# tsbertalan/openmg

Hardware: AMD Instinct MI355X
Metric: V-cycles/sec, 3-D 7-point Poisson 256^3 (higher is better)
Workload: dtype f64

## Files before the change

### include/openmg_hip.h

```cpp
#ifndef OPENMG_HIP_H
#define OPENMG_HIP_H

#include <stdint.h>

#ifdef __cplusplus
extern "C" {
#endif

#define OMG_OK                0
#define OMG_ERR_INVALID       1
#define OMG_ERR_NO_DEVICE     2
#define OMG_ERR_HIP           3
#define OMG_ERR_SINGULAR      4
#define OMG_ERR_NO_DIAGONAL   5
#define OMG_ERR_ALLOC         6
#define OMG_ERR_UNSUPPORTED   7

#define OMG_SMOOTH_GS_LEX     0
#define OMG_SMOOTH_GS_COLOUR  1
#define OMG_SMOOTH_JACOBI     2

typedef struct {
    int64_t n_rows, n_cols, nnz;
    const int32_t *indptr;
// ... 6 lines not shown

const char *omg_last_error(void);
int omg_device_count(int *count);
int omg_set_device(int device);
int omg_device_mem_info(int64_t *free_bytes, int64_t *total_bytes);
int omg_device_synchronize(void);
const char *omg_version(void);

int omg_hierarchy_create(int n_levels, const omg_csr *A, const omg_csr *R,
                         int smoother, double omega, omg_hierarchy **out);
#define OMG_DTYPE_F64 0
#define OMG_DTYPE_F32 1
int omg_hierarchy_create_ex(int n_levels, const omg_csr *A, const omg_csr *R, int smoother,
                            double omega, int dtype, omg_hierarchy **out);
int omg_hierarchy_create_from_fine(const omg_csr *A_in, int dim, const int64_t *shape, int n_restrictions, int smoother, double omega,
                                   int dtype, omg_hierarchy **out);

int omg_hierarchy_update_fine(omg_hierarchy *h, const double *data, int64_t nnz, int on_device);
int omg_hierarchy_dtype(const omg_hierarchy *h, int *dtype);
int omg_hierarchy_destroy(omg_hierarchy *h);
int omg_hierarchy_set_stream(omg_hierarchy *h, void *hip_stream);
int omg_hierarchy_sync(omg_hierarchy *h);
int omg_hierarchy_level_rows(const omg_hierarchy *h, int level, int64_t *n_rows);
int omg_hierarchy_level_sets(const omg_hierarchy *h, int level, int64_t *n_sets);
int omg_hierarchy_level_fused(const omg_hierarchy *h, int level, int *fused);
#define OMG_LEVEL_FUSED_LAST_SET   1
#define OMG_LEVEL_SCATTER_PROLONG  2
#define OMG_LEVEL_UNION_WALK       16
#define OMG_LEVEL_MARCH            32
#define OMG_LEVEL_MARCH_SCAN       512
#define OMG_LEVEL_PLANE            64
#define OMG_LEVEL_VAR7             256
#define OMG_LEVEL_STENCIL27        128
int omg_hierarchy_level_flags(const omg_hierarchy *h, int level, int *flags);
int omg_hierarchy_use_plane(omg_hierarchy *h, int enable);
int omg_hierarchy_plane_info(const omg_hierarchy *h, int level, int64_t *out8);
int omg_hierarchy_set_info(const omg_hierarchy *h, int level, int set, int64_t *rows, int64_t *nnz);
#define OMG_FORMAT_FIELDS 12
int omg_hierarchy_format_info(const omg_hierarchy *h, int level, int op, int set, int64_t *out);
int omg_format_selftest(const omg_csr *A, int dtype, int64_t *out);

int omg_vcycle(omg_hierarchy *h, int level, const double *b, double *x,
               int pre, int post, double *norm);
int omg_vcycle_ex(omg_hierarchy *h, int level, const double *b, const double *x_in, double *x_out, double *x_pre,
                  int pre, int post, double *norm);

int omg_solve(omg_hierarchy *h, const double *b, double *x, int pre, int post,
              int max_cycles, double threshold, int *cycles_done, double *norm);

int omg_vcycle_dev(omg_hierarchy *h, int level, const double *b_dev, const double *x_in_dev, double *x_out_dev,
                   double *x_pre_dev, int pre, int post, double *norm);
int omg_resident_load_dev(omg_hierarchy *h, const double *b_dev, const double *x0_dev );
int omg_resident_fetch_dev(omg_hierarchy *h, double *x_dev);

int omg_hierarchy_cycle_dev(omg_hierarchy *h, const double *b_dev, double *x_dev, int pre, int post,
                            void *hip_stream);

int omg_resident_load(omg_hierarchy *h, const double *b, const double *x0 );
int omg_resident_cycle(omg_hierarchy *h, int pre, int post, double *norm );
int omg_resident_cycles(omg_hierarchy *h, int pre, int post, int n_cycles, double *norms );
int omg_resident_fetch(omg_hierarchy *h, double *x);
int omg_resident_spmv_time(omg_hierarchy *h, int reps, double *avg_ms);
int omg_resident_use_graph(omg_hierarchy *h, int enable);

#define OMG_PROFILE_CLASSES 7
int omg_profile_enable(omg_hierarchy *h, int mask);
// ... 135 lines not shown
```

### openmg_amd/_hip.py

```python
import ctypes
import os

import numpy as np
import scipy.sparse as sp

_HERE = os.path.dirname(os.path.abspath(__file__))
LIB_PATH = os.environ.get("OMG_LIB_PATH") or os.path.join(_HERE, "lib", "libopenmg_hip.so")

OMG_OK = 0
ERR_INVALID, ERR_NO_DEVICE, ERR_HIP, ERR_SINGULAR, ERR_NO_DIAGONAL, ERR_ALLOC, ERR_UNSUPPORTED = range(1, 8)
SMOOTH_GS_LEX, SMOOTH_GS_COLOUR, SMOOTH_JACOBI = 0, 1, 2
PROFILE_CLASSES = 7
PROFILE_NAMES = ("smoother_set_sweep", "residual", "restrict", "prolong_add", "residual_norm", "plane_down", "plane_up")

SMOOTHERS = {
    "gs": SMOOTH_GS_LEX, "lex": SMOOTH_GS_LEX, "gauss-seidel": SMOOTH_GS_LEX, "gaussSeidel": SMOOTH_GS_LEX,
    "colour": SMOOTH_GS_COLOUR, "color": SMOOTH_GS_COLOUR, "rbgs": SMOOTH_GS_COLOUR,
    "red-black": SMOOTH_GS_COLOUR, "multicolour": SMOOTH_GS_COLOUR,
    "jacobi": SMOOTH_JACOBI, "weighted-jacobi": SMOOTH_JACOBI,
}


class HipError(RuntimeError):

# ... 385 lines not shown
        ms = ctypes.c_double(0.0)
        check(lib().omg_resident_spmv_time(self._h, int(reps), ctypes.byref(ms)))
        return ms.value

    def use_graph(self, enable=True):
        check(lib().omg_resident_use_graph(self._h, 1 if enable else 0))

    def set_stream(self, hip_stream):
        check(lib().omg_hierarchy_set_stream(self._h, ctypes.c_void_p(hip_stream or 0)))

    def sync(self):
        check(lib().omg_hierarchy_sync(self._h))

    def device_dtype(self):
        code = ctypes.c_int(-1)
        check(lib().omg_hierarchy_dtype(self._h, ctypes.byref(code)))
        return np.dtype(np.float32 if code.value == DTYPE_F32 else np.float64)

    def level_sets(self, level):
        v = ctypes.c_int64(0)
        check(lib().omg_hierarchy_level_sets(self._h, level, ctypes.byref(v)))
        return v.value

    def level_fused(self, level):
        v = ctypes.c_int(0)
        check(lib().omg_hierarchy_level_fused(self._h, level, ctypes.byref(v)))
        return bool(v.value)

    def level_flags(self, level):
        f = ctypes.c_int(0)
        check(lib().omg_hierarchy_level_flags(self._h, int(level), ctypes.byref(f)))
        return {"fused_last_set": bool(f.value & 1), "scatter_prolong": bool(f.value & 2), "union_walk": bool(f.value & 16),
                "march": bool(f.value & 32), "plane": bool(f.value & 64), "stencil27": bool(f.value & 128), "var7": bool(f.value & 256),
                "march_scan": bool(f.value & 512)}

    def use_plane(self, enable=True):
        check(lib().omg_hierarchy_use_plane(self._h, 1 if enable else 0))

    PLANE_FIELDS = ("nx", "ny", "nz", "tile_x", "tile_y", "tile_z", "workgroups", "threads")

    def plane_info(self, level):
        out = (ctypes.c_int64 * len(self.PLANE_FIELDS))()
        check(lib().omg_hierarchy_plane_info(self._h, int(level), out))
        return dict(zip(self.PLANE_FIELDS, [int(v) for v in out]))

    def set_info(self, level, s):
        rows, nnz = ctypes.c_int64(0), ctypes.c_int64(0)
        check(lib().omg_hierarchy_set_info(self._h, level, s, ctypes.byref(rows), ctypes.byref(nnz)))
        return rows.value, nnz.value

    FORMAT_FIELDS = ("rows", "nnz", "blocks", "pattern_blocks", "pattern_rows", "pattern_nnz",
                     "coldict_nnz", "valdict_nnz", "format_bytes", "csr_bytes", "ell_blocks", "ell_nnz")

    def format_info(self, level, op="A", set=-1):
        out = (ctypes.c_int64 * len(self.FORMAT_FIELDS))()
        check(lib().omg_hierarchy_format_info(self._h, int(level), {"A": 0, "R": 1, "P": 2}[op], int(set), out))
        return dict(zip(self.FORMAT_FIELDS, [int(v) for v in out]))

    def profile_enable(self, classes=True):
        if classes is True:
            mask = -1
        elif not classes:
            mask = 0
        else:
            mask = 0
            for name in classes:
                mask |= 1 << PROFILE_NAMES.index(name)
# ... 147 lines not shown
```

### openmg_amd/csrc/common.h

```cpp
#pragma once
#include <hip/hip_runtime.h>

#include <cstdint>
#include <cstdio>
#include <cstdlib>
#include <stdexcept>
#include <memory>
#include <string>
#include <utility>
#include <vector>

#include "../../include/openmg_hip.h"

#if !defined(OMG_EXPERIMENTS) && (defined(PLANE_STORE_AUX) || defined(PLANE_LA_BIG) || defined(PLANE_LA) || defined(PLANE_WAVE_SYNC) || \
                                  defined(PLANE_WSYNC_F32) || defined(S27_COEF_AUX) || defined(S27_SG) || defined(S27_WAVES) ||        \
                                  defined(MARCH_NAP_MAX) || defined(OMG_ROWBLK_NNZ) || defined(PLANE_SETPRIO))
#error "tuning switches are experiments: add -DOMG_EXPERIMENTS"
#endif

namespace omg {

inline const char *experiment_env(const char *name) {
#ifdef OMG_EXPERIMENTS
    return getenv(name);
// ... 373 lines not shown
    bool build(const omg_csr &A, hipStream_t s);
    void sweep(V *x, const V *b, hipStream_t s) const;
    bool timed_out(hipStream_t s) const;
};

struct DevCsrPlain {
    int64_t n_rows = 0, n_cols = 0, nnz = 0;
    DevBuf<int32_t> indptr, indices;
    DevBuf<double> data;
};
void galerkin_chain_device(const omg_csr &A0, int dim, const int64_t *shape, int n_restrictions, std::vector<DevCsrPlain> &A,
                           std::vector<DevCsrPlain> &R, hipStream_t s);
HostCsr download_csr(const DevCsrPlain &M, hipStream_t s);
bool rap_aggregation_device(const DevCsrPlain &R, const DevCsrPlain &A, DevCsrPlain &C, hipStream_t s);

bool is_plain_aggregation(const omg_csr &R, int64_t nx, int64_t ny, int64_t nz, double &w);

constexpr int PLANE_EDGE = 4;
struct PlaneGeom {
    int nx = 0, ny = 0, nz = 0;
    int hx = 0;
    int z_base = 0, z_end = 0, kv0 = 0, kv1 = 0, kc_off = 0, nzc = 0;
    int TX = 0, TY = 0, LZ = 0;
    int PX = 0, PY = 0;
    int ntx = 0, nty = 0, ntz = 0, n_wg = 0;
    int threads = 0;
    size_t lds_bytes = 0;
    double c[7] = {0, 0, 0, 0, 0, 0, 0};
    double w = 0.0;
    bool dim2 = false;
    bool jacobi = false;
    double omega = 1.0;
    bool block = false;
    bool la2 = true;
};
template <typename V>
struct PlanePlan {
    PlaneGeom g;
    DevBuf<double> partials;
    uint32_t *status = nullptr;
    bool build(const omg_csr &A, const omg_csr &R, Ordering &ord, bool jacobi = false, double omega = 1.0);
    bool build_device(const DevCsrPlain &A, int nx, int ny, int nz, double w, Ordering &ord, bool jacobi, double omega, hipStream_t s);
    bool finish_geometry(int64_t nx, int64_t ny, int64_t nz, const double (&c)[7], double w, bool jacobi, double omega);
    void spmv(const V *x, V *y, hipStream_t s) const;
    HostCsr operator_csr() const;
    HostCsr restriction_csr() const;
    void build_slab(int nx, int ny, int nz_own, int ghost, int ghost_c, bool first, bool last, const double (&c)[7], double w);
    struct Peer {
        V *x[2] = {nullptr, nullptr};
        V *bc[2] = {nullptr, nullptr};
        int64_t shift = 0, cshift = 0;
        int planes = 0, cplanes = 0;
        int zc_lo = 0, zc_hi = 0;
        const uint32_t *wait_flag[4] = {nullptr, nullptr, nullptr, nullptr};
        uint32_t wait_seq[4] = {0, 0, 0, 0};
        bool fused_wait = true;
        uint32_t *done = nullptr;
        uint32_t *flag[2] = {nullptr, nullptr};
        uint32_t seq = 0;
        uint32_t *status = nullptr;
        uint32_t spin = 1u << 21;
    };
    struct Coarse {
        const int32_t *map = nullptr;
        V *b = nullptr;
        V *x = nullptr;
        const V *diag = nullptr;
        int first_end = 0;
        const V *e = nullptr;
    };
    void tune(V *x, V *tmp, const V *b, const Coarse &c, hipStream_t s, bool finest = true);
    float time_pair(V *x, V *tmp, const V *b, const Coarse &c, hipStream_t s, bool finest, int pairs);
    enum { PART_ALL = 0, PART_EDGE = 1, PART_INNER = 2 };
    bool can_split() const {
        return !g.dim2 && !g.block && !(g.la2 && g.threads <= 128) && (g.z_end - g.z_base) >= 3 * PLANE_EDGE;
    }
    int split_partials() const {
        const int nzo = g.z_end - g.z_base;
        return nzo >= 3 * PLANE_EDGE ? g.ntx * g.nty * (2 + (nzo - 2 * PLANE_EDGE + g.LZ - 1) / g.LZ) : g.n_wg;
    }
    struct Gate {
        const uint32_t *flag[4] = {nullptr, nullptr, nullptr, nullptr};
        uint32_t seq[4] = {0, 0, 0, 0};
        uint32_t *status = nullptr;
        uint32_t spin = 1u << 21;
    };
    bool can_gate() const { return can_split() && 2 * g.ntx * g.nty <= 192 && (g.z_end - g.z_base) >= 96; }
    int gate_lz() const;
    int gate_partials() const;
    void down(const V *x_old, V *x_new, const V *b, bool x_zero, const Coarse &c, hipStream_t s, const Peer *peer = nullptr,
              bool sweep = true, int part = PART_ALL, const Gate *gate = nullptr) const;
    void up(const V *x_old, V *x_new, const V *b, const Coarse &c, double *out, hipStream_t s, const Peer *peer = nullptr,
            bool sweep = true, int part = PART_ALL, const Gate *gate = nullptr) const;
};

template <typename V>
struct Var7Plan {
    int nx = 0, ny = 0, nz = 0;
    double w = 0.0;
    bool sym = false;
    int tx = 0, ty = 0, lz = 0, ntx = 0, nty = 0, ntz = 0, threads = 0;
    int64_t n_wg = 0;
    DevBuf<V> cD, cM[3], cP[3];
    DevBuf<double> partials;
// ... 51 lines not shown
```

### openmg_amd/csrc/hierarchy.hip

```cpp
#include <algorithm>
#include <chrono>
#include <cmath>
#include <cstring>
#include <memory>
#include <array>
#include <map>
#include <mutex>
#include <thread>
#include <type_traits>

#include "common.h"

namespace omg {

std::vector<ScatteredBlock> &scattered_registry() {
    static std::vector<ScatteredBlock> r;
    return r;
}
static std::mutex &scattered_mutex() {
    static std::mutex m;
    return m;
}
static void scattered_release(ScatteredBlock &blk, size_t mapped) {
    auto report = [](const char *what, hipError_t e) {
// ... 1544 lines not shown
        with(h, [&](auto *hh) {
            check_level(hh, level);
            OMG_REQUIRE(n_sets, "null");
            *n_sets = (int64_t)hh->lv[level].ord.sets.size() - 1;
        });
    });
}

int omg_hierarchy_level_fused(const omg_hierarchy *h, int level, int *fused) {
    return guarded([&] {
        with(h, [&](auto *hh) {
            check_level(hh, level);
            OMG_REQUIRE(fused, "null");
            ensure_format(hh, level);
            *fused = (level + 1 < (int)hh->lv.size() && can_fuse(hh, hh->lv[level])) ? 1 : 0;
        });
    });
}

int omg_hierarchy_level_flags(const omg_hierarchy *h, int level, int *flags) {
    return guarded([&] {
        with(h, [&](auto *hh) {
            check_level(hh, level);
            OMG_REQUIRE(flags, "null");
            ensure_format(hh, level);
            const bool smoothed = level + 1 < (int)hh->lv.size();
            *flags = ((smoothed && can_fuse(hh, hh->lv[level])) ? OMG_LEVEL_FUSED_LAST_SET : 0) |
                     ((smoothed && hh->lv[level].scatter_prolong) ? OMG_LEVEL_SCATTER_PROLONG : 0) |
                     ((smoothed && hh->lv[level].A.all_union()) ? OMG_LEVEL_UNION_WALK : 0) |
                     ((smoothed && hh->lv[level].march) ? OMG_LEVEL_MARCH : 0) |
                     ((smoothed && hh->lv[level].march && hh->lv[level].march->line_scan) ? OMG_LEVEL_MARCH_SCAN : 0) |
                     ((smoothed && hh->lv[level].plane && !hh->no_plane) ? OMG_LEVEL_PLANE : 0) |
                     ((smoothed && hh->lv[level].s27 && !hh->no_plane) ? OMG_LEVEL_STENCIL27 : 0) |
                     ((smoothed && hh->lv[level].var7 && !hh->no_plane) ? OMG_LEVEL_VAR7 : 0);
        });
    });
}

int omg_hierarchy_use_plane(omg_hierarchy *h, int enable) {
    return guarded([&] {
        with(h, [&](auto *hh) {
            OMG_HIP(hipStreamSynchronize(hh->stream));
            drop_graph(hh);
            hh->no_plane = enable == 0;
        });
    });
}

int omg_hierarchy_plane_info(const omg_hierarchy *h, int level, int64_t *out8) {
    return guarded([&] {
        with(h, [&](auto *hh) {
            check_level(hh, level);
            OMG_REQUIRE(out8, "null");
            for (int i = 0; i < 8; ++i) out8[i] = 0;
            const auto &L = hh->lv[level];
            if (!L.plane) return;
            const PlaneGeom &g = L.plane->g;
            const int64_t v[8] = {g.nx, g.ny, g.nz, g.TX, g.TY, g.LZ, g.n_wg, g.threads};
            for (int i = 0; i < 8; ++i) out8[i] = v[i];
        });
    });
}

int omg_hierarchy_set_info(const omg_hierarchy *h, int level, int set, int64_t *rows, int64_t *nnz) {
    return guarded([&] {
        with(h, [&](auto *hh) {
            check_level(hh, level);
// ... 690 lines not shown
```

### openmg_amd/csrc/plane.hip

```cpp
#include <algorithm>
#include <array>
#include <atomic>
#include <cmath>
#include <cstring>
#include <map>
#include <mutex>
#include <thread>
#include <type_traits>

#include "common.h"

#if defined(OMG_PLANE_STAMPS) || defined(OMG_PLANE_DBGARGS)
#define OMG_PLANE_DBG_ON 1
#endif

namespace omg {
namespace {

#ifndef PLANE_STORE_AUX
#define PLANE_STORE_AUX 2
#endif
typedef unsigned v2u __attribute__((ext_vector_type(2)));
typedef unsigned v4u __attribute__((ext_vector_type(4)));
typedef int v2i __attribute__((ext_vector_type(2)));
// ... 1029 lines not shown
            E[c] = B[l] - row(l);
            if (SWEEP) a.x_new[slot_of(gi, gj, gk)] = X[l];
        }
        __syncthreads();
#pragma unroll
        for (int n = 0; n < NC; ++n) {
            const int c = t + n * NT;
            if (cs[n] < 0) continue;
            const int I = c % hx, J = (c / hx) % hy, K = c / (hx * hy);
            V acc = V(0);
#pragma unroll
            for (int d = 0; d < 8; ++d)
                acc = madd(a.w, E[((2 * K + (d >> 2)) * BY + 2 * J + ((d >> 1) & 1)) * BX + 2 * I + (d & 1)], acc);
            a.bc[cs[n]] = acc;
        }
    } else {
        if (SWEEP) {
            sweep(0, R1(), std::false_type());
            __syncthreads();
            sweep(1, R0(), std::false_type());
            __syncthreads();
        }
#pragma unroll
        for (int n = 0; n < NB; ++n) {
            const int c = t + n * NT;
            const int li = 2 + c % BX, lj = 2 + (c / BX) % BY, lk = 2 + c / (BX * BY);
            const int gi = i0 + li, gj = j0 + lj, gk = k0 + lk;
            if (c >= BX * BY * BZ || gi >= a.nx || gj >= a.ny || gk >= a.nz) continue;
            a.x_new[slot_of(gi, gj, gk)] = X[(lk * EY + lj) * EX + li];
        }
    }
}

template <typename V>
struct Tile2KArgs {
    const V *x_old;
    V *x_new;
    const V *b;
    int nx, ny, nr;
    int nbx;
    V c1, c2, c3, c4, c5, w, omega;
    int fast_div;
    int nxc, nyc;
    const int32_t *cmap;
    V *bc;
    const V *ec;
    double *partials;
};

template <typename V, int MODE, bool XZ, bool NORM, bool SWEEP, int BX, int BY, bool JAC = false>
__global__ __launch_bounds__(256) void tile2d_kernel(const Tile2KArgs<V> a) {
    extern __shared__ __attribute__((aligned(16))) unsigned char plane_smem[];
    constexpr int EX = BX + 6, EY = BY + 6, vol = EX * EY, NT = 256;
    V *const X = reinterpret_cast<V *>(plane_smem);
    V *const B = X + vol;
    V *const XN = B + vol;
    V *const E = JAC ? XN + vol : XN;
    __shared__ double s_red[NT / 64];
    const int t = int(threadIdx.x);
    const int bi = int(blockIdx.x) % a.nbx, bj = int(blockIdx.x) / a.nbx;
    const int i0 = bi * BX - 3, j0 = bj * BY - 3;
    const V rc3 = refined_rcp(a.c3);
    const bool fast = a.fast_div != 0;
    auto slot_of = [&](int gi, int gj) { return JAC ? gj * a.nx + gi : (((gi + gj) & 1) ? a.nr : 0) + ((gj * a.nx + gi) >> 1); };
    auto in_grid = [&](int gi, int gj) { return gi >= 0 && gi < a.nx && gj >= 0 && gj < a.ny; };
    constexpr int NL = (vol + NT - 1) / NT;
// ... 102 lines not shown
        for (int n = 0; n < NCC; ++n) {
            const int c = t + n * NT;
            const int I = c % hx, J = c / hx;
            const int GI = (bi * BX >> 1) + I, GJ = (bj * BY >> 1) + J;
            if (c >= hx * hy || GI >= a.nxc || GJ >= a.nyc) continue;
            V acc = V(0);
#pragma unroll
            for (int d = 0; d < 4; ++d) acc = madd(a.w, E[(2 * J + (d >> 1)) * BX + 2 * I + (d & 1)], acc);
            const int ce = GJ * a.nxc + GI;
            a.bc[a.cmap ? a.cmap[ce] : ce] = acc;
        }
    }
    if (NORM) {
#pragma unroll
        for (int off = 32; off > 0; off >>= 1) sq += __shfl_down(sq, off, 64);
        if ((t & 63) == 0) s_red[t >> 6] = sq;
        __syncthreads();
        if (t == 0) {
            double tot = 0.0;
            for (int wv = 0; wv < NT / 64; ++wv) tot += s_red[wv];
            a.partials[blockIdx.x] = tot;
        }
    }
}

int env_int3(const char *name, int out[3]) {
    const char *e = getenv(name);
    if (!e || !e[0]) return 0;
    return sscanf(e, "%d,%d,%d", &out[0], &out[1], &out[2]) == 3 ? 1 : 0;
}

inline int round_up(int v, int m) { return (v + m - 1) / m * m; }

inline void small_level_switches(PlaneGeom &g) {
    auto env = [](const char *name, long long dflt) { const char *e = getenv(name); return e && e[0] ? atoll(e) : dflt; };
    const bool whole = g.z_base == 0 && g.z_end == g.nz && g.kv0 == 0 && g.kv1 == g.nz;
    g.block = env("OMG_PLANE_BLOCK", 1) != 0 && whole && int64_t(g.nx) * g.ny * g.nz <= env("OMG_PLANE_BLOCK_CELLS", int64_t(64) * 64 * 64);
    g.la2 = env("OMG_PLANE_LA2", 1) != 0;
}

void choose_tiles(PlaneGeom &g, size_t value_bytes, int model = 0, std::vector<std::array<int, 3>> *more = nullptr, int keep = 0) {
    const int nzo = g.z_end - g.z_base;
    auto set = [&](int TX, int TY, int LZ) {
        g.TX = TX; g.TY = TY; g.LZ = LZ;
        g.PX = TX / 4 + 2; g.PY = TY / 2 + 4;
        g.ntx = (g.nx + TX - 1) / TX; g.nty = (g.ny + TY - 1) / TY; g.ntz = (nzo + LZ - 1) / LZ;
        g.n_wg = g.ntx * g.nty * g.ntz;
        g.threads = round_up(g.PX * g.PY, 64);
        g.lds_bytes = size_t(6) * size_t(2 * g.PY + 2) * size_t(2 * g.PX + 4) * value_bytes;
    };
    int forced[3];
    if (env_int3("OMG_PLANE_TILE", forced)) {
        const int TX = std::max(4, round_up(forced[0], 4)), TY = std::max(2, round_up(forced[1], 2)), LZ = std::max(2, round_up(forced[2], 2));
        set(TX, TY, LZ);
        if (g.threads <= 512 && g.lds_bytes <= size_t(160) * 1024) return;
    }
    std::vector<std::pair<double, std::array<int, 3>>> all;
    for (int ntx = 1; ntx <= (g.nx + 3) / 4; ++ntx) {
        const int TX = round_up((g.nx + ntx - 1) / ntx, 4);
        if ((g.nx + TX - 1) / TX != ntx) continue;
        for (int nty = 1; nty <= g.ny / 2; ++nty) {
            const int TY = round_up((g.ny + nty - 1) / nty, 2);
            if ((g.ny + TY - 1) / TY != nty) continue;
            const int thr = round_up((TX / 4 + 2) * (TY / 2 + 4), 64);
            if (thr > 512) continue;
            if (size_t(6) * size_t(TY + 10) * size_t(TX / 2 + 8) * value_bytes > size_t(150) * 1024) continue;
            for (int ntz = 1; ntz <= nzo / 2; ++ntz) {
                const int LZ = round_up((nzo + ntz - 1) / ntz, 2);
                if ((nzo + LZ - 1) / LZ != ntz) continue;
                double cost;
// ... 279 lines not shown
    if (jacobi) {
        ord.identity = true;
        ord.sets = {0, n};
    } else {
        ord.identity = false;
        ord.sets = {0, n / 2, n};
        ord.closed_form = 2; ord.cf_nx = nx; ord.cf_ny = ny; ord.cf_nz = nz;
    }
    return finish_geometry(nx, ny, nz, c, w, jacobi, omega);
}

template <typename V>
void PlanePlan<V>::build_slab(int nx, int ny, int nz_own, int ghost, int ghost_c, bool first, bool last, const double (&c)[7], double w) {
    OMG_REQUIRE(nx >= 2 && ny >= 2 && nz_own >= 2 && !(nx & 1) && !(ny & 1) && !(nz_own & 1) && !(ghost & 1) && ghost >= 4 && ghost_c >= 2,
                "plane slab: extents must be even, at least four ghost planes (two on the coarse slab)");
    g = PlaneGeom();
    g.nx = nx; g.ny = ny; g.nz = nz_own + 2 * ghost; g.hx = nx / 2;
    for (int e = 0; e < 7; ++e) g.c[e] = double(V(c[e]));
    g.w = double(V(w));
    g.z_base = ghost; g.z_end = ghost + nz_own;
    g.kv0 = first ? ghost : 0;
    g.kv1 = last ? ghost + nz_own : g.nz;
    g.nzc = nz_own / 2 + 2 * ghost_c;
    g.kc_off = ghost_c - ghost / 2;
    OMG_REQUIRE(uint64_t(nx) * ny * g.nz * sizeof(V) < (uint64_t(1) << 31), "plane slab: vector exceeds 2 GiB");
    choose_tiles(g, sizeof(V));
    small_level_switches(g);
    OMG_REQUIRE(g.TX > 0 && g.threads <= 512, "plane slab: no tiling");
    partials.alloc(size_t(std::max(g.n_wg, split_partials())) + SUM_FOLD);
}

template <typename V>
void PlanePlan<V>::tune(V *x, V *tmp, const V *b, const Coarse &c, hipStream_t s, bool finest) {
    {
        const char *e = experiment_env("OMG_PLANE_TUNE");
        int forced[3];
        if ((e && e[0] == '0') || env_int3("OMG_PLANE_TILE", forced)) return;
    }
    if (g.dim2 || int64_t(g.nx) * g.ny * (g.z_end - g.z_base) < (int64_t(1) << 21)) return;
    static const int keep = [] { const char *e = experiment_env("OMG_PLANE_TUNE_K"); return e ? std::max(0, atoi(e)) : 0; }();
    static const bool debug = [] { const char *e = experiment_env("OMG_PLANE_TUNE_DEBUG"); return e && e[0] == '1'; }();
    std::vector<PlaneGeom> cand;
    {
        std::vector<std::array<int, 3>> more0, more1;
        PlaneGeom g0 = g, g1 = g;
        choose_tiles(g0, sizeof(V), 0, &more0, keep);
        choose_tiles(g1, sizeof(V), 1, &more1, keep);
        auto add = [&](const PlaneGeom &q) {
            if (q.TX <= 0 || q.threads > 512) return;
            for (const PlaneGeom &c : cand)
                if (c.TX == q.TX && c.TY == q.TY && c.LZ == q.LZ) return;
            cand.push_back(q);
        };
        add(g);
        add(g0);
        add(g1);
        auto from = [&](const std::array<int, 3> &t) {
            PlaneGeom q = g;
            q.TX = t[0]; q.TY = t[1]; q.LZ = t[2];
            q.PX = q.TX / 4 + 2; q.PY = q.TY / 2 + 4;
            const int nzo = q.z_end - q.z_base;
            q.ntx = (q.nx + q.TX - 1) / q.TX; q.nty = (q.ny + q.TY - 1) / q.TY; q.ntz = (nzo + q.LZ - 1) / q.LZ;
            q.n_wg = q.ntx * q.nty * q.ntz;
            q.threads = round_up(q.PX * q.PY, 64);
            q.lds_bytes = size_t(6) * size_t(2 * q.PY + 2) * size_t(2 * q.PX + 4) * sizeof(V);
            return q;
// ... 206 lines not shown
            what, g.nx, g.ny, g.nz, g.n_wg, g.threads, m / steps, tp / steps, sB / steps, sC / steps, c / steps, b / steps);
}
#endif

template <typename K>
void allow_lds(K kernel, size_t bytes) {
    if (bytes > size_t(64) * 1024)
        OMG_HIP(hipFuncSetAttribute(reinterpret_cast<const void *>(kernel), hipFuncAttributeMaxDynamicSharedMemorySize, int(bytes)));
}

}

template <typename V>
void peer_args(PlaneKArgs<V> &k, const typename PlanePlan<V>::Peer &p, hipStream_t s) {
    for (int i = 0; i < 2; ++i) { k.peer_x[i] = p.x[i]; k.peer_bc[i] = p.bc[i]; k.peer_flag[i] = p.flag[i]; }
    k.peer_shift = int(p.shift); k.peer_cshift = int(p.cshift);
    OMG_REQUIRE(p.planes == PEER_PLANES && (p.cplanes == PEER_CPLANES || (!p.bc[0] && !p.bc[1])), "plane pass with neighbours: three planes of x, two of the coarse right-hand side");
    for (int i = 0; i < 4; ++i) { k.wait_flag[i] = p.wait_flag[i]; k.wait_seq[i] = p.wait_seq[i]; }
    k.fused_wait = p.fused_wait ? 1 : 0;
    k.done = p.done; k.flag_seq = p.seq; k.status = p.status; k.spin = p.spin;
    OMG_REQUIRE(p.done, "plane pass with neighbours: no workgroup counter");
    if (!p.fused_wait && (p.wait_flag[0] || p.wait_flag[1] || p.wait_flag[2] || p.wait_flag[3])) {
        hipLaunchKernelGGL(plane_wait_kernel, dim3(1), dim3(64), 0, s, p.wait_flag[0], p.wait_flag[1], p.wait_flag[2], p.wait_flag[3],
                           p.wait_seq[0], p.wait_seq[1], p.wait_seq[2], p.wait_seq[3], p.status, p.spin);
        OMG_HIP(hipGetLastError());
    }
}

struct BlockGeom {
    int shape, BX, BY, BZ, nbx, nby, nbz, threads;
    size_t lds;
};
inline bool block_level(const PlaneGeom &g) { return g.block; }
constexpr int BLOCK_SHAPES[4][3] = {{16, 8, 8}, {8, 8, 8}, {8, 4, 4}, {4, 4, 4}};
inline BlockGeom choose_block(const PlaneGeom &g, size_t value_bytes) {
    BlockGeom k;
    int pick = 3;
    for (int i = 0; i < 4; ++i) {
        const int64_t n = int64_t((g.nx + BLOCK_SHAPES[i][0] - 1) / BLOCK_SHAPES[i][0]) * ((g.ny + BLOCK_SHAPES[i][1] - 1) / BLOCK_SHAPES[i][1]) *
                          ((g.nz + BLOCK_SHAPES[i][2] - 1) / BLOCK_SHAPES[i][2]);
        if (n >= 128) { pick = i; break; }
    }
    k.shape = pick;
    k.BX = BLOCK_SHAPES[pick][0]; k.BY = BLOCK_SHAPES[pick][1]; k.BZ = BLOCK_SHAPES[pick][2];
    k.nbx = (g.nx + k.BX - 1) / k.BX; k.nby = (g.ny + k.BY - 1) / k.BY; k.nbz = (g.nz + k.BZ - 1) / k.BZ;
    const size_t vol = size_t(k.BX + 4) * size_t(k.BY + 4) * size_t(k.BZ + 4);
    k.threads = vol >= 1024 ? 256 : 128;
    k.lds = (2 * vol + std::max(size_t(k.BX) * k.BY * k.BZ, vol / 8)) * value_bytes;
    return k;
}
template <typename V, int MODE, int S, bool SWEEP>
void launch_block_shape(const BlockGeom &k, const BlockKArgs<V> &a, hipStream_t s) {
    auto kernel = block_kernel<V, MODE, BLOCK_SHAPES[S][0], BLOCK_SHAPES[S][1], BLOCK_SHAPES[S][2], SWEEP>;
    allow_lds(kernel, k.lds);
    hipLaunchKernelGGL(kernel, dim3(unsigned(k.nbx * k.nby * k.nbz)), dim3(unsigned(k.threads)), k.lds, s, a);
}
template <typename V, int MODE, bool SWEEP = true>
void launch_block(const PlaneGeom &g, const V *x_old, V *x_new, const V *b, const typename PlanePlan<V>::Coarse &c, hipStream_t s) {
    const BlockGeom k = choose_block(g, sizeof(V));
    BlockKArgs<V> a;
    std::memset(&a, 0, sizeof(a));
    a.x_old = x_old; a.x_new = x_new; a.b = b;
    a.nx = g.nx; a.ny = g.ny; a.nz = g.nz; a.nr = int(int64_t(g.nx) * g.ny * g.nz / 2);
    a.nbx = k.nbx; a.nby = k.nby;
    a.c0 = V(g.c[0]); a.c1 = V(g.c[1]); a.c2 = V(g.c[2]); a.c3 = V(g.c[3]); a.c4 = V(g.c[4]); a.c5 = V(g.c[5]); a.c6 = V(g.c[6]);
    a.w = V(g.w);
    a.fast_div = (std::fabs(g.c[3]) >= 0x1p-400 && std::fabs(g.c[3]) <= 0x1p400) ? 1 : 0;
    a.nxc = g.nx / 2; a.nyc = g.ny / 2;
    a.cmap = c.map; a.bc = c.b; a.ec = c.e;
    switch (k.shape) {
        case 0: launch_block_shape<V, MODE, 0, SWEEP>(k, a, s); break;
        case 1: launch_block_shape<V, MODE, 1, SWEEP>(k, a, s); break;
        case 2: launch_block_shape<V, MODE, 2, SWEEP>(k, a, s); break;
        default: launch_block_shape<V, MODE, 3, SWEEP>(k, a, s); break;
    }
    OMG_HIP(hipGetLastError());
}


template <typename V, int MODE, bool XZ, bool NORM, bool SWEEP>
void launch_tile2d(const PlaneGeom &g, const V *x_old, V *x_new, const V *b, const typename PlanePlan<V>::Coarse &c, double *out, hipStream_t s) {
    Tile2KArgs<V> a;
    std::memset(&a, 0, sizeof(a));
    a.x_old = x_old; a.x_new = x_new; a.b = b;
    a.nx = g.nx; a.ny = g.ny; a.nr = int(int64_t(g.nx) * g.ny / 2);
    a.nbx = g.ntx;
    a.c1 = V(g.c[1]); a.c2 = V(g.c[2]); a.c3 = V(g.c[3]); a.c4 = V(g.c[4]); a.c5 = V(g.c[5]);
    a.w = V(g.w);
    a.omega = V(g.omega);
    a.fast_div = (std::fabs(g.c[3]) >= 0x1p-400 && std::fabs(g.c[3]) <= 0x1p400) ? 1 : 0;
    a.nxc = g.nx / 2; a.nyc = g.ny / 2;
    a.cmap = c.map; a.bc = c.b; a.ec = c.e;
    a.partials = out;
    auto go = [&](auto kernel) {
        allow_lds(kernel, g.lds_bytes);
        hipLaunchKernelGGL(kernel, dim3(unsigned(g.n_wg)), dim3(256), g.lds_bytes, s, a);
    };
    if (g.jacobi) {
        if (g.TX == 64) go(tile2d_kernel<V, MODE, XZ, NORM, SWEEP, 64, 32, true>);
        else if (g.TX == 32) go(tile2d_kernel<V, MODE, XZ, NORM, SWEEP, 32, 16, true>);
        else go(tile2d_kernel<V, MODE, XZ, NORM, SWEEP, 16, 8, true>);
    } else {
        if (g.TX == 64) go(tile2d_kernel<V, MODE, XZ, NORM, SWEEP, 64, 32>);
        else if (g.TX == 32) go(tile2d_kernel<V, MODE, XZ, NORM, SWEEP, 32, 16>);
        else go(tile2d_kernel<V, MODE, XZ, NORM, SWEEP, 16, 8>);
    }
    OMG_HIP(hipGetLastError());
// ... 78 lines not shown
    } else if (!peer && x_zero && !c.x && !c.diag && block_level(g)) {
        launch_block<V, 0>(g, x_old, x_new, b, c, s);
    } else if (peer) {
        peer_args<V>(k, *peer, s);
        if (x_zero) launch_plane(plane_kernel<V, 0, false, true, PLANE_LA, true>, g, k, s);
        else launch_plane(plane_kernel<V, 0, false, false, PLANE_LA, true>, g, k, s);
    } else if (c.x || c.diag) {
        if (x_zero) launch_plane(plane_kernel<V, 0, false, true, PLANE_LA, false, 512, true>, g, k, s);
        else launch_plane(plane_kernel<V, 0, false, false, PLANE_LA, false, 512, true>, g, k, s);
    } else if (small_tile(g)) {
        if (x_zero) launch_plane(plane_kernel<V, 0, false, true, 2, false, 128>, g, k, s);
        else launch_plane(plane_kernel<V, 0, false, false, 2, false, 128>, g, k, s);
    } else if (x_zero) {
        launch_plane(plane_kernel<V, 0, false, true, PLANE_LA_BIG>, g, k, s, wgs);
    } else {
        launch_plane(plane_kernel<V, 0, false, false, PLANE_LA_BIG>, g, k, s, wgs);
    }
#ifdef OMG_PLANE_STAMPS
    stamps_end("down", g, sb, s);
#endif
}

template <typename V>
void PlanePlan<V>::up(const V *x_old, V *x_new, const V *b, const Coarse &c, double *out, hipStream_t s, const Peer *peer, bool sweep, int part,
                      const Gate *gate) const {
    PlaneKArgs<V> k = plane_args<V>(g, x_old, x_new, b, c, status);
    k.partials = out;
    OMG_REQUIRE(part == 0 || (!peer && sweep && !g.dim2 && !block_level(g) && !(small_tile(g) && !out)),
                "a pass in two launches: slabs' marching passes only");
    OMG_REQUIRE(!gate || (part == 0 && !peer && sweep && can_gate()), "a gated pass: thick slabs' marching passes only");
    const int wgs = gate ? plane_gate<V>(g, k, *gate, gate_lz()) : plane_part(g, k, part);
    const char *mirror_env = getenv("OMG_PLANE_MIRROR");
    const bool mirror_on = !(mirror_env && mirror_env[0] == '0');
    const bool mirror = mirror_on && !peer && part == 0 && !g.dim2 && !block_level(g) && !small_tile(g) && (g.nz & 1) == 0 && g.z_base == g.nz - g.z_end;
    if (mirror) { k.kv0 = g.nz - g.kv1; k.kv1 = g.nz - g.kv0; }
#ifdef OMG_PLANE_STAMPS
    DevBuf<unsigned long long> sb;
    stamps_begin(k, g, sb);
#endif
    if (g.dim2) {
        OMG_REQUIRE(!peer, "2-D plane level: no slab neighbours");
        if (sweep) {
            if (out) launch_tile2d<V, 1, false, true, true>(g, x_old, x_new, b, c, out, s);
            else launch_tile2d<V, 1, false, false, true>(g, x_old, x_new, b, c, nullptr, s);
        } else {
            if (out) launch_tile2d<V, 1, false, true, false>(g, x_old, x_new, b, c, out, s);
            else launch_tile2d<V, 1, false, false, false>(g, x_old, x_new, b, c, nullptr, s);
        }
    } else if (!sweep) {
        OMG_REQUIRE(!peer, "plane pass without its sweep: not built for slabs with neighbours");
        if (!out && block_level(g)) launch_block<V, 1, false>(g, x_old, x_new, b, c, s);
        else if (mirror && out) launch_plane(plane_kernel<V, 1, true, false, PLANE_LA, false, 512, false, false, true>, g, k, s);
        else if (mirror) launch_plane(plane_kernel<V, 1, false, false, PLANE_LA, false, 512, false, false, true>, g, k, s);
        else if (out) launch_plane(plane_kernel<V, 1, true, false, PLANE_LA, false, 512, false, false>, g, k, s);
        else launch_plane(plane_kernel<V, 1, false, false, PLANE_LA, false, 512, false, false>, g, k, s);
    } else if (!peer && !out && block_level(g)) {
        launch_block<V, 1>(g, x_old, x_new, b, c, s);
    } else if (peer) {
        peer_args<V>(k, *peer, s);
        if (out) launch_plane(plane_kernel<V, 1, true, false, PLANE_LA, true>, g, k, s);
        else launch_plane(plane_kernel<V, 1, false, false, PLANE_LA, true>, g, k, s);
    } else if (small_tile(g) && !out) {
        launch_plane(plane_kernel<V, 1, false, false, 2, false, 128>, g, k, s);
    } else if (mirror) {
        if (out) launch_plane(plane_kernel<V, 1, true, false, PLANE_LA_BIG, false, 512, false, true, true>, g, k, s, wgs);
        else launch_plane(plane_kernel<V, 1, false, false, PLANE_LA_BIG, false, 512, false, true, true>, g, k, s, wgs);
    } else if (out) {
        launch_plane(plane_kernel<V, 1, true, false, PLANE_LA_BIG>, g, k, s, wgs);
    } else {
        launch_plane(plane_kernel<V, 1, false, false, PLANE_LA_BIG>, g, k, s, wgs);
    }
#ifdef OMG_PLANE_STAMPS
    stamps_end("up", g, sb, s);
#endif
}

template <typename V>
void PlanePlan<V>::spmv(const V *x, V *y, hipStream_t s) const {
    OMG_REQUIRE(!g.jacobi && g.z_base == 0 && g.z_end == g.nz, "matrix-free SpMV: whole red-black ordered grids only");
    PlaneSpmvArgs<V> a;
    std::memset(&a, 0, sizeof(a));
    const int64_t n = int64_t(g.nx) * g.ny * g.nz;
    a.x = x; a.y = y;
    a.vec_bytes = unsigned(n * int64_t(sizeof(V)));
    a.nr = int(n / 2); a.hx = g.hx; a.ny = g.ny; a.nz = g.nz; a.hq = (g.hx + 1) / 2;
    a.c0 = V(g.c[0]); a.c1 = V(g.c[1]); a.c2 = V(g.c[2]); a.c3 = V(g.c[3]); a.c4 = V(g.c[4]); a.c5 = V(g.c[5]); a.c6 = V(g.c[6]);
    static const int mode = [] { const char *e = getenv("OMG_PLANE_SPMV"); return e ? atoi(e) : 1; }();
    static const int lz_env = [] { const char *e = getenv("OMG_PLANE_SPMV_LZ"); return e ? atoi(e) : 0; }();
    if (mode != 0 && a.hq <= 256) {
// ... 27 lines not shown
```

Baseline: 3531.

## Add large-block smoother kernel for mid-size levels, chosen by setup-time timing

Adds a 1024-thread block kernel working on 32x16x16 tiles held in LDS. It fuses the red-black sweep with restriction on the way down, and prolongation with the sweep on the way up. Levels between 64^3 and 128^3 cells now time three options at setup: the marching kernels, blocks for both passes, or blocks only for the down pass. The fastest is kept. This aims to cut the cost of marching kernels on mid-size coarse levels, at the price of setup timing, redundant halo work and high LDS and register use per workgroup.

```diff
diff --git a/include/openmg_hip.h b/include/openmg_hip.h
--- a/include/openmg_hip.h
+++ b/include/openmg_hip.h
@@ -62,6 +62,8 @@
 #define OMG_LEVEL_PLANE            64
 #define OMG_LEVEL_VAR7             256
 #define OMG_LEVEL_STENCIL27        128
+#define OMG_LEVEL_PLANE_BLOCK      1024
+#define OMG_LEVEL_PLANE_BLOCK_TIMED 2048
 int omg_hierarchy_level_flags(const omg_hierarchy *h, int level, int *flags);
 int omg_hierarchy_use_plane(omg_hierarchy *h, int enable);
 int omg_hierarchy_plane_info(const omg_hierarchy *h, int level, int64_t *out8);
diff --git a/openmg_amd/_hip.py b/openmg_amd/_hip.py
--- a/openmg_amd/_hip.py
+++ b/openmg_amd/_hip.py
@@ -441,7 +441,8 @@
         check(lib().omg_hierarchy_level_flags(self._h, int(level), ctypes.byref(f)))
         return {"fused_last_set": bool(f.value & 1), "scatter_prolong": bool(f.value & 2), "union_walk": bool(f.value & 16),
                 "march": bool(f.value & 32), "plane": bool(f.value & 64), "stencil27": bool(f.value & 128), "var7": bool(f.value & 256),
-                "march_scan": bool(f.value & 512)}
+                "march_scan": bool(f.value & 512),
+                "plane_block": bool(f.value & 1024), "plane_block_timed": bool(f.value & 2048)}
 
     def use_plane(self, enable=True):
         check(lib().omg_hierarchy_use_plane(self._h, 1 if enable else 0))
diff --git a/openmg_amd/csrc/common.h b/openmg_amd/csrc/common.h
--- a/openmg_amd/csrc/common.h
+++ b/openmg_amd/csrc/common.h
@@ -429,6 +429,8 @@
     bool jacobi = false;
     double omega = 1.0;
     bool block = false;
+    bool block_up = true;
+    bool block_try = false;
     bool la2 = true;
 };
 template <typename V>
@@ -467,6 +469,7 @@
         const V *e = nullptr;
     };
     void tune(V *x, V *tmp, const V *b, const Coarse &c, hipStream_t s, bool finest = true);
+    void tune_tiles(V *x, V *tmp, const V *b, const Coarse &c, hipStream_t s, bool finest);
     float time_pair(V *x, V *tmp, const V *b, const Coarse &c, hipStream_t s, bool finest, int pairs);
     enum { PART_ALL = 0, PART_EDGE = 1, PART_INNER = 2 };
     bool can_split() const {
diff --git a/openmg_amd/csrc/hierarchy.hip b/openmg_amd/csrc/hierarchy.hip
--- a/openmg_amd/csrc/hierarchy.hip
+++ b/openmg_amd/csrc/hierarchy.hip
@@ -1600,7 +1600,9 @@
                      ((smoothed && hh->lv[level].march && hh->lv[level].march->line_scan) ? OMG_LEVEL_MARCH_SCAN : 0) |
                      ((smoothed && hh->lv[level].plane && !hh->no_plane) ? OMG_LEVEL_PLANE : 0) |
                      ((smoothed && hh->lv[level].s27 && !hh->no_plane) ? OMG_LEVEL_STENCIL27 : 0) |
-                     ((smoothed && hh->lv[level].var7 && !hh->no_plane) ? OMG_LEVEL_VAR7 : 0);
+                     ((smoothed && hh->lv[level].var7 && !hh->no_plane) ? OMG_LEVEL_VAR7 : 0) |
+                     ((smoothed && hh->lv[level].plane && !hh->no_plane && hh->lv[level].plane->g.block) ? OMG_LEVEL_PLANE_BLOCK : 0) |
+                     ((smoothed && hh->lv[level].plane && !hh->no_plane && hh->lv[level].plane->g.block_try) ? OMG_LEVEL_PLANE_BLOCK_TIMED : 0);
         });
     });
 }
diff --git a/openmg_amd/csrc/plane.hip b/openmg_amd/csrc/plane.hip
--- a/openmg_amd/csrc/plane.hip
+++ b/openmg_amd/csrc/plane.hip
@@ -1085,6 +1085,164 @@
     }
 }
 
+template <typename V, int MODE, int BX, int BY, int BZ, bool SWEEP = true>
+__global__ __launch_bounds__(1024) void block_big_kernel(const BlockKArgs<V> a) {
+    extern __shared__ __attribute__((aligned(16))) unsigned char plane_smem[];
+    constexpr int EX = BX + 4, EY = BY + 4, EZ = BZ + 4, vol = EX * EY * EZ, NT = 1024;
+    V *const X = reinterpret_cast<V *>(plane_smem);
+    V *const E = X + vol;
+    const int t = int(threadIdx.x);
+    const int bi = int(blockIdx.x) % a.nbx, bj = (int(blockIdx.x) / a.nbx) % a.nby, bk = int(blockIdx.x) / (a.nbx * a.nby);
+    const int i0 = bi * BX - 2, j0 = bj * BY - 2, k0 = bk * BZ - 2;
+    constexpr int CX = EX / 2, CY = EY / 2, CZ = EZ / 2;
+    constexpr int hx = BX / 2, hy = BY / 2, hz = BZ / 2;
+    const int ci0 = i0 >> 1, cj0 = j0 >> 1, ck0 = k0 >> 1;
+    const int nzc = a.nz >> 1;
+    const V rc3 = refined_rcp(a.c3);
+    const bool fast = a.fast_div != 0;
+    auto slot_of = [&](int gi, int gj, int gk) { return (((gi + gj + gk) & 1) ? a.nr : 0) + (((gk * a.ny + gj) * a.nx + gi) >> 1); };
+    auto in_grid = [&](int gi, int gj, int gk) { return gi >= 0 && gi < a.nx && gj >= 0 && gj < a.ny && gk >= 0 && gk < a.nz; };
+    auto row = [&](int c) -> V {
+        V s = madd(a.c0, X[c - EX * EY], V(0));
+        s = madd(a.c1, X[c - EX], s);
+        s = madd(a.c2, X[c - 1], s);
+        s = madd(a.c3, X[c], s);
+        s = madd(a.c4, X[c + 1], s);
+        s = madd(a.c5, X[c + EX], s);
+        return madd(a.c6, X[c + EX * EY], s);
+    };
+    auto pairs = [](int ring) { return (BX + 2 * ring) / 2 * (BY + 2 * ring) * (BZ + 2 * ring); };
+    auto pair_cell = [&](int p, int colour, int ring, V &bv) -> int {
+        const int wx = BX + 2 * ring, wy = BY + 2 * ring, off = 2 - ring;
+        const int lj = off + (p / (wx / 2)) % wy, lk = off + p / (wx / 2 * wy);
+        const int li = off + 2 * (p % (wx / 2)) + ((off + lj + lk + colour) & 1);
+        const int gi = i0 + li, gj = j0 + lj, gk = k0 + lk;
+        const bool ok = p < pairs(ring) && in_grid(gi, gj, gk);
+        bv = a.b[ok ? slot_of(gi, gj, gk) : 0];
+        return ok ? (lk * EY + lj) * EX + li : -1;
+    };
+    auto relax = [&](int l, V bv) { X[l] = X[l] + block_quotient(bv - row(l), a.c3, rc3, fast); };
+
+    if (MODE == 0) {
+        constexpr int N2 = (EX / 2 * EY * EZ + NT - 1) / NT, N1 = ((BX + 2) / 2 * (BY + 2) * (BZ + 2) + NT - 1) / NT;
+        constexpr int NC = (hx * hy * hz + NT - 1) / NT;
+        int cs[NC];
+        V b2[SWEEP ? N2 : 1], b1[SWEEP ? N1 : 1], b0[NC][8];
+        int l2[SWEEP ? N2 : 1], l1[SWEEP ? N1 : 1];
+        if (SWEEP) {
+#pragma unroll
+            for (int n = 0; n < N2; ++n) l2[n] = pair_cell(t + n * NT, 0, 2, b2[n]);
+#pragma unroll
+            for (int n = 0; n < N1; ++n) l1[n] = pair_cell(t + n * NT, 1, 1, b1[n]);
+        }
+#pragma unroll
+        for (int n = 0; n < NC; ++n) {
+            const int c = t + n * NT;
+            const int I = (bi * BX >> 1) + c % hx, J = (bj * BY >> 1) + (c / hx) % hy, K = (bk * BZ >> 1) + c / (hx * hy);
+            const bool ok = c < hx * hy * hz && I < a.nxc && J < a.nyc && K < nzc;
+            const int ce = (K * a.nyc + J) * a.nxc + I;
+            cs[n] = ok ? (a.cmap ? a.cmap[ce] : ce) : -1;
+#pragma unroll
+            for (int d = 0; d < 8; ++d)
+                b0[n][d] = a.b[ok ? slot_of(2 * I + (d & 1), 2 * J + ((d >> 1) & 1), 2 * K + (d >> 2)) : 0];
+        }
+#pragma unroll
+        for (int n = 0; n < N2; ++n) {
+            const int p = t + n * NT;
+            if (p >= EX / 2 * EY * EZ) continue;
+            const int lj = (p / (EX / 2)) % EY, lk = p / (EX / 2 * EY);
+            const int lr = 2 * (p % (EX / 2)) + ((lj + lk) & 1);
+            X[(lk * EY + lj) * EX + (lr ^ 1)] = V(0);
+            X[(lk * EY + lj) * EX + lr] =SWEEP && l2[n] >= 0 ? V(0) + block_quotient(b2[n] - V(0), a.c3, rc3, fast) : V(0);
+        }
+        __syncthreads();
+        if (SWEEP) {
+#pragma unroll
+            for (int n = 0; n < N1; ++n)
+                if (l1[n] >= 0) relax(l1[n], b1[n]);
+            __syncthreads();
+        }
+#pragma unroll
+        for (int n = 0; n < NC; ++n) {
+            if (cs[n] < 0) continue;
+            const int c = t + n * NT;
+            const int I = c % hx, J = (c / hx) % hy, K = c / (hx * hy);
+            V acc = V(0);
+#pragma unroll
+            for (int d = 0; d < 8; ++d) {
+                const int li = 2 + 2 * I + (d & 1), lj = 2 + 2 * J + ((d >> 1) & 1), lk = 2 + 2 * K + (d >> 2);
+                const int l = (lk * EY + lj) * EX + li;
+                const V res = b0[n][d] - row(l);
+                acc = madd(a.w, res, acc);
+                if (SWEEP) a.x_new[slot_of(i0 + li, j0 + lj, k0 + lk)] = X[l];
+            }
+            a.bc[cs[n]] = acc;
+        }
+    } else {
+        constexpr int NL = (vol + NT - 1) / NT, NE = (CX * CY * CZ + NT - 1) / NT;
+        constexpr int N1 = ((BX + 2) / 2 * (BY + 2) * (BZ + 2) + NT - 1) / NT, N0 = (BX / 2 * BY * BZ + NT - 1) / NT;
+        V xv[NL], ev[NE], b1[SWEEP ? N1 : 1], b0[SWEEP ? N0 : 1];
+        int l1[SWEEP ? N1 : 1], l0[SWEEP ? N0 : 1];
+#pragma unroll
+        for (int n = 0; n < NL; ++n) {
+            const int c = t + n * NT;
+            const int gi = i0 + c % EX, gj = j0 + (c / EX) % EY, gk = k0 + c / (EX * EY);
+            const bool ok = c < vol && in_grid(gi, gj, gk);
+            xv[n] = a.x_old[ok ? slot_of(gi, gj, gk) : 0];
+            if (!ok) xv[n] = V(0);
+        }
+#pragma unroll
+        for (int n = 0; n < NE; ++n) {
+            const int c = t + n * NT;
+            const int I = ci0 + c % CX, J = cj0 + (c / CX) % CY, K = ck0 + c / (CX * CY);
+            const bool ok = c < CX * CY * CZ && I >= 0 && J >= 0 && K >= 0 && I < a.nxc && J < a.nyc && K < nzc;
+            const int ce = (K * a.nyc + J) * a.nxc + I;
+            const int cs = ok ? (a.cmap ? a.cmap[ce] : ce) : -1;
+            ev[n] = a.ec[cs >= 0 ? cs : 0];
+            if (cs < 0) ev[n] = V(0);
+        }
+        if (SWEEP) {
+#pragma unroll
+            for (int n = 0; n < N1; ++n) l1[n] = pair_cell(t + n * NT, 0, 1, b1[n]);
+#pragma unroll
+            for (int n = 0; n < N0; ++n) l0[n] = pair_cell(t + n * NT, 1, 0, b0[n]);
+        }
+#pragma unroll
+        for (int n = 0; n < NE; ++n)
+            if (t + n * NT < CX * CY * CZ) E[t + n * NT] = ev[n];
+        int tt = t;
+        asm volatile("" : "+v"(tt));
+        __syncthreads();
+#pragma unroll
+        for (int n = 0; n < NL; ++n) {
+            const int c = tt + n * NT;
+            if (c >= vol) continue;
+            const int li = c % EX, lj = (c / EX) % EY, lk = c / (EX * EY);
+            X[c] = in_grid(i0 + li, j0 + lj, k0 + lk) ? xv[n] + madd(a.w, E[((lk >> 1) * CY + (lj >> 1)) * CX + (li >> 1)], V(0)) : V(0);
+        }
+        __syncthreads();
+        if (SWEEP) {
+#pragma unroll
+            for (int n = 0; n < N1; ++n)
+                if (l1[n] >= 0) relax(l1[n], b1[n]);
+            __syncthreads();
+#pragma unroll
+            for (int n = 0; n < N0; ++n)
+                if (l0[n] >= 0) relax(l0[n], b0[n]);
+            __syncthreads();
+        }
+        constexpr int NB = (BX * BY * BZ + NT - 1) / NT;
+#pragma unroll
+        for (int n = 0; n < NB; ++n) {
+            const int c = tt + n * NT;
+            const int li = 2 + c % BX, lj = 2 + (c / BX) % BY, lk = 2 + c / (BX * BY);
+            const int gi = i0 + li, gj = j0 + lj, gk = k0 + lk;
+            if (c >= BX * BY * BZ || gi >= a.nx || gj >= a.ny || gk >= a.nz) continue;
+            a.x_new[slot_of(gi, gj, gk)] = X[(lk * EY + lj) * EX + li];
+        }
+    }
+}
+
 template <typename V>
 struct Tile2KArgs {
     const V *x_old;
@@ -1253,10 +1411,14 @@
 
 inline int round_up(int v, int m) { return (v + m - 1) / m * m; }
 
+constexpr int64_t BLOCK_BIG_ABOVE = int64_t(64) * 64 * 64;
 inline void small_level_switches(PlaneGeom &g) {
     auto env = [](const char *name, long long dflt) { const char *e = getenv(name); return e && e[0] ? atoll(e) : dflt; };
     const bool whole = g.z_base == 0 && g.z_end == g.nz && g.kv0 == 0 && g.kv1 == g.nz;
-    g.block = env("OMG_PLANE_BLOCK", 1) != 0 && whole && int64_t(g.nx) * g.ny * g.nz <= env("OMG_PLANE_BLOCK_CELLS", int64_t(64) * 64 * 64);
+    const int64_t cells = int64_t(g.nx) * g.ny * g.nz;
+    g.block = env("OMG_PLANE_BLOCK", 1) != 0 && whole && cells <= env("OMG_PLANE_BLOCK_CELLS", BLOCK_BIG_ABOVE);
+    const bool forced = env("OMG_PLANE_BLOCK", -1) != -1 || env("OMG_PLANE_BLOCK_CELLS", -1) != -1;
+    g.block_try = !forced && whole && !g.dim2 && cells > BLOCK_BIG_ABOVE && cells <= int64_t(128) * 128 * 128;
     g.la2 = env("OMG_PLANE_LA2", 1) != 0;
 }
 
@@ -1602,6 +1764,29 @@
 
 template <typename V>
 void PlanePlan<V>::tune(V *x, V *tmp, const V *b, const Coarse &c, hipStream_t s, bool finest) {
+    const bool block = g.block;
+    g.block = false;
+    tune_tiles(x, tmp, b, c, s, finest);
+    g.block = block;
+    if (finest || experiment_flag0("OMG_PLANE_TUNE")) g.block_try = false;
+    if (!g.block_try) return;
+    float us[3] = {0.0f, 0.0f, 0.0f};
+    for (int r = 0; r < 3; ++r)
+        for (int f = 0; f < 3; ++f) {
+            g.block = f >= 1;
+            g.block_up = f == 1;
+            us[f] += time_pair(x, tmp, b, c, s, false, 2);
+        }
+    const int pick = us[2] < us[1] ? (us[2] < us[0] ? 2 : 0) : (us[1] < us[0] ? 1 : 0);
+    g.block = pick >= 1;
+    g.block_up = pick == 1;
+    if (SetupTimer::on())
+        fprintf(stderr, "[omg setup] %dx%dx%d level: marching %7.1f us, block_big_kernel %7.1f us, down as blocks + up marching %7.1f us per down + up: %s\n",
+                g.nx, g.ny, g.nz, us[0] / 3, us[1] / 3, us[2] / 3, pick == 0 ? "marching" : pick == 1 ? "blocks" : "down as blocks");
+}
+
+template <typename V>
+void PlanePlan<V>::tune_tiles(V *x, V *tmp, const V *b, const Coarse &c, hipStream_t s, bool finest) {
     {
         const char *e = experiment_env("OMG_PLANE_TUNE");
         int forced[3];
@@ -1874,9 +2059,19 @@
     size_t lds;
 };
 inline bool block_level(const PlaneGeom &g) { return g.block; }
-constexpr int BLOCK_SHAPES[4][3] = {{16, 8, 8}, {8, 8, 8}, {8, 4, 4}, {4, 4, 4}};
+inline bool block_up_level(const PlaneGeom &g) { return g.block && g.block_up; }
+constexpr int BLOCK_SHAPES[5][3] = {{16, 8, 8}, {8, 8, 8}, {8, 4, 4}, {4, 4, 4}, {32, 16, 16}};
 inline BlockGeom choose_block(const PlaneGeom &g, size_t value_bytes) {
     BlockGeom k;
+    if (int64_t(g.nx) * g.ny * g.nz > BLOCK_BIG_ABOVE) {
+        k.shape = 4;
+        k.BX = BLOCK_SHAPES[4][0]; k.BY = BLOCK_SHAPES[4][1]; k.BZ = BLOCK_SHAPES[4][2];
+        k.nbx = (g.nx + k.BX - 1) / k.BX; k.nby = (g.ny + k.BY - 1) / k.BY; k.nbz = (g.nz + k.BZ - 1) / k.BZ;
+        const size_t vol = size_t(k.BX + 4) * size_t(k.BY + 4) * size_t(k.BZ + 4);
+        k.threads = 1024;
+        k.lds = (vol + vol / 8) * value_bytes;
+        return k;
+    }
     int pick = 3;
     for (int i = 0; i < 4; ++i) {
         const int64_t n = int64_t((g.nx + BLOCK_SHAPES[i][0] - 1) / BLOCK_SHAPES[i][0]) * ((g.ny + BLOCK_SHAPES[i][1] - 1) / BLOCK_SHAPES[i][1]) *
@@ -1893,7 +2088,9 @@
 }
 template <typename V, int MODE, int S, bool SWEEP>
 void launch_block_shape(const BlockGeom &k, const BlockKArgs<V> &a, hipStream_t s) {
-    auto kernel = block_kernel<V, MODE, BLOCK_SHAPES[S][0], BLOCK_SHAPES[S][1], BLOCK_SHAPES[S][2], SWEEP>;
+    void (*kernel)(BlockKArgs<V>);
+    if constexpr (S == 4) kernel = block_big_kernel<V, MODE, BLOCK_SHAPES[S][0], BLOCK_SHAPES[S][1], BLOCK_SHAPES[S][2], SWEEP>;
+    else kernel = block_kernel<V, MODE, BLOCK_SHAPES[S][0], BLOCK_SHAPES[S][1], BLOCK_SHAPES[S][2], SWEEP>;
     allow_lds(kernel, k.lds);
     hipLaunchKernelGGL(kernel, dim3(unsigned(k.nbx * k.nby * k.nbz)), dim3(unsigned(k.threads)), k.lds, s, a);
 }
@@ -1914,7 +2111,8 @@
         case 0: launch_block_shape<V, MODE, 0, SWEEP>(k, a, s); break;
         case 1: launch_block_shape<V, MODE, 1, SWEEP>(k, a, s); break;
         case 2: launch_block_shape<V, MODE, 2, SWEEP>(k, a, s); break;
-        default: launch_block_shape<V, MODE, 3, SWEEP>(k, a, s); break;
+        case 3: launch_block_shape<V, MODE, 3, SWEEP>(k, a, s); break;
+        default: launch_block_shape<V, MODE, 4, SWEEP>(k, a, s); break;
     }
     OMG_HIP(hipGetLastError());
 }
@@ -2059,7 +2257,7 @@
     const int wgs = gate ? plane_gate<V>(g, k, *gate, gate_lz()) : plane_part(g, k, part);
     const char *mirror_env = getenv("OMG_PLANE_MIRROR");
     const bool mirror_on = !(mirror_env && mirror_env[0] == '0');
-    const bool mirror = mirror_on && !peer && part == 0 && !g.dim2 && !block_level(g) && !small_tile(g) && (g.nz & 1) == 0 && g.z_base == g.nz - g.z_end;
+    const bool mirror = mirror_on && !peer && part == 0 && !g.dim2 && !block_up_level(g) && !small_tile(g) && (g.nz & 1) == 0 && g.z_base == g.nz - g.z_end;
     if (mirror) { k.kv0 = g.nz - g.kv1; k.kv1 = g.nz - g.kv0; }
 #ifdef OMG_PLANE_STAMPS
     DevBuf<unsigned long long> sb;
@@ -2076,12 +2274,12 @@
         }
     } else if (!sweep) {
         OMG_REQUIRE(!peer, "plane pass without its sweep: not built for slabs with neighbours");
-        if (!out && block_level(g)) launch_block<V, 1, false>(g, x_old, x_new, b, c, s);
+        if (!out && block_up_level(g)) launch_block<V, 1, false>(g, x_old, x_new, b, c, s);
         else if (mirror && out) launch_plane(plane_kernel<V, 1, true, false, PLANE_LA, false, 512, false, false, true>, g, k, s);
         else if (mirror) launch_plane(plane_kernel<V, 1, false, false, PLANE_LA, false, 512, false, false, true>, g, k, s);
         else if (out) launch_plane(plane_kernel<V, 1, true, false, PLANE_LA, false, 512, false, false>, g, k, s);
         else launch_plane(plane_kernel<V, 1, false, false, PLANE_LA, false, 512, false, false>, g, k, s);
-    } else if (!peer && !out && block_level(g)) {
+    } else if (!peer && !out && block_up_level(g)) {
         launch_block<V, 1>(g, x_old, x_new, b, c, s);
     } else if (peer) {
         peer_args<V>(k, *peer, s);
```

Measured after the change: 3572 (median of 6 runs). 1.01x the previous value.
